# chrg127/stereomatching

Hardware: AMD Instinct MI355X
Metric: Mpixel-disparities/s (higher is better)
Workload: dtype u32 bit-packed edges, i32 counts

## Files before the change

stereomatching_amd/csrc/sm_bs_network.h:

```cpp
#pragma once

#ifdef SM_BS_NETWORK_HOST
#include <cstdint>
typedef uint32_t u32;
#define SM_NET_FN inline
#define SM_NET_UNROLL
#define SM_PIN() do { } while (0)
#define SM_SYNC() do { } while (0)
template <int IMM>
inline u32 bop(u32 a, u32 b, u32 c)
{
    u32 r = 0;
    for (int k = 0; k < 8; k++)
        if ((IMM >> k) & 1) r |= ((k & 4) ? a : ~a) & ((k & 2) ? b : ~b) & ((k & 1) ? c : ~c);
    return r;
}
#else
#define SM_NET_FN __device__ __forceinline__
#define SM_NET_UNROLL _Pragma("unroll")
#endif

#include "sm_bs_ops.h"

struct NetCell { short a, b, c, s, cy; short imm; short w; };

template <int N, int SB>
struct NetPlan {
    static constexpr int NIN = 2 * N + SB;
    static constexpr int MAXC = 2 * N + 2 * SB;
    NetCell cell[MAXC] = {};
    int ncell = 0;
    int nwires = NIN;
    int nops = 0;
    short out[SB] = {};
};

template <int N, int SB>
constexpr NetPlan<N, SB> net_make_plan()
{
    NetPlan<N, SB> p;
    short q[4 * N + 4 * SB] = {}, nx[2 * N + 2 * SB] = {};
    bool qneg[4 * N + 4 * SB] = {}, nxneg[2 * N + 2 * SB] = {};
    int head = 0, tail = 0, nn = 0;
    for (int w = 0; w < SB; w++) {
        const bool top = w == SB - 1;
        head = 0; tail = 0;
        q[tail] = (short)(2 * N + w); qneg[tail++] = false;
        if (w == 0)
            for (int i = 0; i < N; i++) {
                q[tail] = (short)i; qneg[tail++] = false;
                q[tail] = (short)(N + i); qneg[tail++] = true;
            }
        for (int i = 0; i < nn; i++) { q[tail] = nx[i]; qneg[tail++] = nxneg[i]; }
        nn = 0;
        while (tail - head >= 2) {
            const int k = tail - head >= 3 ? 3 : 2;
            short in[3] = {-1, -1, -1};
            int np = 0, ng = 0;
            for (int j = 0; j < k; j++) if (!qneg[head + j]) in[np++] = q[head + j];
            for (int j = 0; j < k; j++) if (qneg[head + j]) in[np + ng++] = q[head + j];
            head += k;
            NetCell c = {in[0], in[1], in[2], (short)p.nwires++, -1, 0, (short)w};
            bool sneg = false, cneg = false;
            if (k == 3) {
                sneg = ng & 1; cneg = ng >= 2;
                c.imm = ng == 1 ? BOP_MAJ_NC : ng == 2 ? BOP_BORROW : BOP_MAJ;
            } else {
                sneg = ng == 2; cneg = ng >= 1;
                c.imm = ng == 1 ? BOP_ANDN : 0;
            }
            p.nops++;
            if (!top) {
                c.cy = (short)p.nwires++;
                nx[nn] = c.cy; nxneg[nn++] = cneg;
                p.nops++;
            }
            q[--head] = c.s; qneg[head] = sneg;
            p.cell[p.ncell++] = c;
        }
        p.out[w] = q[head];
        if (qneg[head] && !top) { nx[nn] = q[head]; nxneg[nn++] = true; }
    }
    bool made[NetPlan<N, SB>::NIN + 2 * NetPlan<N, SB>::MAXC] = {};
    for (int i = 0; i < NetPlan<N, SB>::NIN; i++) made[i] = true;
    NetCell order[NetPlan<N, SB>::MAXC] = {};
    bool done[NetPlan<N, SB>::MAXC] = {};
    for (int n = 0; n < p.ncell; n++) {
        int pick = -1;
        for (int i = 0; i < p.ncell; i++) {
            const NetCell &c = p.cell[i];
            if (done[i] || !made[c.a] || !made[c.b] || (c.c >= 0 && !made[c.c])) continue;
            if (pick < 0 || c.w > p.cell[pick].w) pick = i;
        }
        done[pick] = true;
        order[n] = p.cell[pick];
        made[order[n].s] = true;
        if (order[n].cy >= 0) made[order[n].cy] = true;
    }
    for (int n = 0; n < p.ncell; n++) p.cell[n] = order[n];
    return p;
}

template <int N, int SB>
struct NetPlanOf { static constexpr NetPlan<N, SB> value = net_make_plan<N, SB>(); };

template <int N, int SB>
constexpr int net_min_distance(int it)
{
    const NetPlan<N, SB> p = NetPlanOf<N, SB>::value;
    int pos[NetPlan<N, SB>::NIN + 2 * NetPlan<N, SB>::MAXC] = {};
    for (int i = 0; i < NetPlan<N, SB>::NIN; i++) pos[i] = -(1 << 20);
    int at = 0, best = 1 << 20;
    for (int n = 0; n < p.ncell; n++) {
        const NetCell &c = p.cell[n];
        const short in[3] = {c.a, c.b, c.c};
        for (int j = 0; j < 3; j++)
            if (in[j] >= 0 && at - pos[in[j]] < best) best = at - pos[in[j]];
        pos[c.s] = at; at += it;
        if (c.cy >= 0) { pos[c.cy] = at; at += it; }
    }
    return best;
}

template <int N>
constexpr int net_ops() { return net_make_plan<N, bits_for(N * N)>().nops; }
constexpr int net_ops_count_tree(int n)
{
    int ops = 0, m = n;
    for (int w = 0; w < bits_for(n); w++) {
        int carries = 0;
        while (m >= 3) { ops += 2; m -= 2; carries++; }
        if (m == 2) { ops += 2; m = 1; carries++; }
        m = carries;
    }
    return ops;
}
constexpr int net_ops_addsub(int n)
{
    const int hb = bits_for(n), sb = bits_for(n * n);
    int ops = 2 + 2 * (hb - 1) + 2;
    for (int k = 1; k < sb; k++) ops += k + 1 < sb ? 2 : 1;
    return ops;
}
constexpr int net_ops_separate(int n) { return 2 * net_ops_count_tree(n) + net_ops_addsub(n); }

template <int N, int SB, int IT, int DS, int NW, int ID, typename XF>
SM_NET_FN u32 net_wire(const u32 (&S)[DS][SB], int dd0, XF &xin, const u32 (&wr)[IT][NW], int it)
{
    if constexpr (ID < 2 * N) return xin(it, ID);
    else if constexpr (ID < 2 * N + SB) return S[dd0 + it][ID - 2 * N];
    else return wr[it][ID - 2 * N - SB];
}

template <int N, int SB, int IT, int DS, int C, int NW, typename XF>
SM_NET_FN void net_cells(u32 (&S)[DS][SB], int dd0, XF &xin, u32 (&wr)[IT][NW])
{
    constexpr NetPlan<N, SB> P = NetPlanOf<N, SB>::value;
    if constexpr (C < P.ncell) {
        constexpr NetCell cl = P.cell[C];
        constexpr int NIN = 2 * N + SB;
        constexpr bool full = cl.c >= 0;
        u32 a[IT], b[IT], c[IT];
SM_NET_UNROLL
        for (int it = 0; it < IT; it++) {
            a[it] = net_wire<N, SB, IT, DS, NW, cl.a>(S, dd0, xin, wr, it);
            b[it] = net_wire<N, SB, IT, DS, NW, cl.b>(S, dd0, xin, wr, it);
            if constexpr (full) c[it] = net_wire<N, SB, IT, DS, NW, cl.c>(S, dd0, xin, wr, it);
            else c[it] = 0u;
        }
SM_NET_UNROLL
        for (int it = 0; it < IT; it++) {
            if constexpr (full) wr[it][cl.s - NIN] = bop<BOP_XOR3>(a[it], b[it], c[it]);
            else wr[it][cl.s - NIN] = a[it] ^ b[it];
            SM_PIN();
        }
        if constexpr (cl.cy >= 0) {
SM_NET_UNROLL
            for (int it = 0; it < IT; it++) {
                if constexpr (full || cl.imm != 0) wr[it][cl.cy - NIN] = bop<cl.imm>(a[it], b[it], c[it]);
                else wr[it][cl.cy - NIN] = a[it] & b[it];
                SM_PIN();
            }
        }
        SM_SYNC();
        net_cells<N, SB, IT, DS, C + 1, NW>(S, dd0, xin, wr);
    }
}

template <int N, int SB>
constexpr bool net_planes_from_cells()
{
    constexpr NetPlan<N, SB> P = NetPlanOf<N, SB>::value;
    for (int k = 0; k < SB; k++)
        if (P.out[k] < 2 * N + SB) return false;
    return true;
}

template <int N, int SB, int IT, int DS, typename XF>
SM_NET_FN void network_lockstep(u32 (&S)[DS][SB], int dd0, XF xin)
{
    constexpr NetPlan<N, SB> P = NetPlanOf<N, SB>::value;
    constexpr int NIN = 2 * N + SB, NW = P.nwires - NIN;
    static_assert(net_planes_from_cells<N, SB>(), "every plane of S' comes out of a cell");
    static_assert(net_min_distance<N, SB>(IT) >= IT, "a cell reads a result made fewer than IT operations before");
    u32 wr[IT][NW];
    net_cells<N, SB, IT, DS, 0, NW>(S, dd0, xin, wr);
SM_NET_UNROLL
    for (int k = 0; k < SB; k++)
SM_NET_UNROLL
        for (int it = 0; it < IT; it++) S[dd0 + it][k] = wr[it][P.out[k] - NIN];
}
```

stereomatching_amd/csrc/sm_match_bs_kernel.h:

```cpp

#pragma once
#include "sm_internal.h"

#ifndef SM_BS_TU
#error "define SM_BS_TU (a token naming the translation unit) before including this header"
#endif
#define SM_BS_CAT2(a, b) a##b
#define SM_BS_CAT(a, b) SM_BS_CAT2(a, b)

#define SM_BS_WAVES 2

#ifdef SM_STAMPS
static __device__ unsigned long long *g_sm_stamps;
int SM_BS_CAT(sm_bs_set_stamps_, SM_BS_TU)(void *buf)
{
    return hipMemcpyToSymbol(HIP_SYMBOL(g_sm_stamps), &buf, sizeof buf) == hipSuccess ? 0 : SM_ERR_HIP;
}
#define SM_STAMP(slot)                                                                          \
    do {                                                                                        \
        if ((threadIdx.x & 63) == 0 && g_sm_stamps) {                   \
            const size_t wg_ = (((size_t)blockIdx.z * gridDim.y + blockIdx.y) * gridDim.x + blockIdx.x) \
                               * (blockDim.x >> 6) + (threadIdx.x >> 6);                        \
            g_sm_stamps[wg_ * 10 + 2 * (slot)] = __builtin_amdgcn_s_memrealtime();              \
            g_sm_stamps[wg_ * 10 + 2 * (slot) + 1] = __builtin_amdgcn_s_memtime();              \
            if ((slot) == 0)                                                                    \
                g_sm_stamps[wg_ * 10 + 8] = ((unsigned long long)__builtin_amdgcn_s_getreg(63508) << 32) | \
                                            (unsigned)__builtin_amdgcn_s_getreg(63492);         \
        }                                                                                       \
    } while (0)
#else
#define SM_STAMP(slot) do { } while (0)
#endif

template <int IMM>
__device__ __forceinline__ u32 bop(u32 a, u32 b, u32 c)
{
    return __builtin_amdgcn_bitop3_b32(a, b, c, IMM);
}
#include "sm_bs_ops.h"

__device__ __forceinline__ u32 alignbit(u32 hi, u32 lo, u32 sh)
{
    return __builtin_amdgcn_alignbit(hi, lo, sh);
}

typedef unsigned long long u64;
struct RawRow { u64 l01; u32 l2; u64 r01, r23; };
struct RawCentre { u32 l; u64 r01; u32 r2; };
typedef __attribute__((address_space(3))) const volatile u32 lds_vu32;
typedef u64 __attribute__((aligned(4))) u64a4;
typedef __attribute__((address_space(3))) const volatile u64a4 lds_vu64;
__device__ __forceinline__ void lds_issue(RawRow &o, u32 aL, u32 aR)
{
    o.l01 = *(lds_vu64 *)(uintptr_t)aL;
    o.l2 = *(lds_vu32 *)(uintptr_t)(aL + 8);
    o.r01 = *(lds_vu64 *)(uintptr_t)aR;
    o.r23 = *(lds_vu64 *)(uintptr_t)(aR + 8);
}
__device__ __forceinline__ void lds_issue(RawCentre &o, u32 aL, u32 aR)
{
    o.l = *(lds_vu32 *)(uintptr_t)aL;
    o.r01 = *(lds_vu64 *)(uintptr_t)aR;
    o.r2 = *(lds_vu32 *)(uintptr_t)(aR + 8);
}

typedef int v4i __attribute__((ext_vector_type(4)));
__device__ __forceinline__ void store_map4(i32 *p, v4i v)
{
    asm volatile("global_store_dwordx4 %0, %1, off sc1\n\ts_nop 1" : : "v"(p), "v"(v) : "memory");
}

template <int SB, int HB>
__device__ __forceinline__ void add_planes(u32 (&s)[SB], const u32 (&h)[HB])
{
    u32 c = s[0] & h[0];
    s[0] ^= h[0];
#pragma unroll
    for (int k = 1; k < SB; k++) {
        if (k < HB) {
            const u32 cn = bop<BOP_MAJ>(s[k], h[k], c);
            s[k] = bop<BOP_XOR3>(s[k], h[k], c);
            c = cn;
        } else {
            const u32 cn = k + 1 < SB ? s[k] & c : 0u;
            s[k] ^= c;
            c = cn;
        }
    }
}

#define SM_PIN() __builtin_amdgcn_sched_barrier(0)
#define SM_SYNC() do { asm volatile("s_nop 0"); SM_PIN(); } while (0)

#include "sm_bs_network.h"

template <int N, int HB, int IT, typename XF>
__device__ __forceinline__ void count_lockstep(XF xin, u32 (&h)[IT][HB])
{
    u32 q[IT][2 * N + 2];
    int head = 0, tail = N;
#pragma unroll
    for (int w = 0; w < HB; w++) {
        u32 nx[IT][N + 1];
        int nn = 0;
#pragma unroll
        for (int adder = 0; adder < N; adder++) {
            if (tail - head >= 3) {
                u32 a[IT], b[IT], c[IT];
#pragma unroll
                for (int it = 0; it < IT; it++) {
                    const bool in0 = w == 0 && head < N, in1 = w == 0 && head + 1 < N, in2 = w == 0 && head + 2 < N;
                    a[it] = in0 ? xin(it, in0 ? head : 0) : q[it][head];
                    b[it] = in1 ? xin(it, in1 ? head + 1 : 0) : q[it][head + 1];
                    c[it] = in2 ? xin(it, in2 ? head + 2 : 0) : q[it][head + 2];
                }
#pragma unroll
                for (int it = 0; it < IT; it++) { q[it][tail] = bop<BOP_XOR3>(a[it], b[it], c[it]); SM_PIN(); }
#pragma unroll
                for (int it = 0; it < IT; it++) { nx[it][nn] = bop<BOP_MAJ>(a[it], b[it], c[it]); SM_PIN(); }
                SM_SYNC();
                head += 3; tail++; nn++;
            }
        }
        if (tail - head == 2) {
            u32 a[IT], b[IT];
#pragma unroll
            for (int it = 0; it < IT; it++) {
                const bool in0 = w == 0 && head < N, in1 = w == 0 && head + 1 < N;
                a[it] = in0 ? xin(it, in0 ? head : 0) : q[it][head];
                b[it] = in1 ? xin(it, in1 ? head + 1 : 0) : q[it][head + 1];
            }
#pragma unroll
            for (int it = 0; it < IT; it++) { q[it][tail] = a[it] ^ b[it]; SM_PIN(); }
#pragma unroll
            for (int it = 0; it < IT; it++) { nx[it][nn] = a[it] & b[it]; SM_PIN(); }
            head += 2; tail++; nn++;
        }
#pragma unroll
        for (int it = 0; it < IT; it++) {
            const bool in0 = w == 0 && head < N;
            h[it][w] = tail - head == 1 ? (in0 ? xin(it, in0 ? head : 0) : q[it][head]) : 0u;
        }
        head = 0; tail = 0;
#pragma unroll
        for (int i = 0; i < N + 1; i++)
            if (i < nn) {
#pragma unroll
                for (int it = 0; it < IT; it++) q[it][tail] = nx[it][i];
                tail++;
            }
    }
}

template <int SB, int HB, int GS, int DS>
__device__ __forceinline__ void add_lockstep(u32 (&S)[DS][SB], int dd0, const u32 (&h)[GS][HB])
{
    u32 c[GS];
#pragma unroll
    for (int g = 0; g < GS; g++) { c[g] = S[dd0 + g][0] & h[g][0]; SM_PIN(); }
#pragma unroll
    for (int g = 0; g < GS; g++) { S[dd0 + g][0] ^= h[g][0]; SM_PIN(); }
#pragma unroll
    for (int k = 1; k < SB; k++) {
        u32 cn[GS];
#pragma unroll
        for (int g = 0; g < GS; g++) {
            if (k + 1 < SB) { cn[g] = k < HB ? bop<BOP_MAJ>(S[dd0 + g][k], h[g][k], c[g]) : (S[dd0 + g][k] & c[g]); SM_PIN(); }
            else cn[g] = 0;
        }
#pragma unroll
        for (int g = 0; g < GS; g++) {
            if (k < HB) S[dd0 + g][k] = bop<BOP_XOR3>(S[dd0 + g][k], h[g][k], c[g]);
            else S[dd0 + g][k] ^= c[g];
            SM_PIN();
        }
#pragma unroll
        for (int g = 0; g < GS; g++) c[g] = cn[g];
        SM_SYNC();
    }
}

template <int V> struct IntTag { static constexpr int value = V; };

template <int CTRL>
__device__ __forceinline__ u32 dpp(u32 v)
{
    return (u32)__builtin_amdgcn_update_dpp(0, (int)v, CTRL, 0xf, 0xf, true);
}

template <int K>
__device__ __forceinline__ u32 from_partner(u32 v)
{
    if (K == 0) return dpp<0xB1>(v);
    if (K == 1) return dpp<0x4E>(v);
    if (K == 2) return dpp<0x141>(v);
    if (K == 3) return dpp<0x140>(v);
    return (u32)__shfl_xor((int)v, 1 << K);
}


template <int N, int DS, bool FULLD, bool GHOST, bool CAP2 = false, bool DUO = false>
__global__ __launch_bounds__(DUO ? 128 : 64, SM_BS_WAVES) void k_match_bs(const u32 *__restrict__ ext,
                                                 i32 *__restrict__ web, i32 *__restrict__ best,
                                                 const MatchGeom g)
{
    constexpr int HALF = N / 2;
    constexpr int HB = bits_for(N);
    constexpr int SB = bits_for(N * N);
    constexpr int AB = DS == 16 ? 4 : DS == 8 ? 3 : 2;
    constexpr int ABMAX = AB + 6;
    static_assert(SB <= 16, "window counts are moved through two byte lanes");
    static_assert((1 << SB) - 1 > N * N, "the all-ones marker must not be a real count");
    static_assert(N + DS - 1 + 31 < 96, "right window must fit three words");

    extern __shared__ __attribute__((aligned(16))) u32 lds[];
    if (CAP2) asm volatile("" ::: "v175");
    if (web == nullptr) return;
    const int tid = DUO ? (int)(threadIdx.x & 63u) : (int)threadIdx.x;
    const int wv = DUO ? __builtin_amdgcn_readfirstlane((int)(threadIdx.x >> 6)) : 0;
    const int pair = blockIdx.z;
    SM_STAMP(0);
    const unsigned slot_parity = __builtin_amdgcn_s_getreg(63492) & 1;
    unsigned long long clk = __builtin_amdgcn_s_memtime();
    constexpr unsigned PATTERN = DS == 16 ? 0xF0F0F0F0u : 0xAAAAAAAAu;
    const unsigned long long clk0 = clk;
#define SM_SLICE_PRIO()                                                               \
    do {                                                                              \
        const unsigned unit_ = (unsigned)((clk - clk0) >> 14) & 31u;                  \
        if (((PATTERN >> unit_) ^ slot_parity) & 1) __builtin_amdgcn_s_setprio(3);    \
        else __builtin_amdgcn_s_setprio(0);                                           \
    } while (0)
#define SM_SLICE_READ() do { clk = __builtin_amdgcn_s_memtime(); } while (0)
    int tile_x, tile_y;
    sm_xcd_tile(g.tiles_x, g.tiles_y, tile_x, tile_y);
    const int tx0 = tile_x * g.tw;
    const int ty0 = tile_y * (DUO ? 2 * g.tile_h : g.tile_h);
    const int plw = g.plw, prw = g.prw, nsr = g.nsr;
    const u32 *extL = ext + (size_t)pair * 2 * g.ext_image_words;
    const u32 *extR = extL + g.ext_image_words;
    u32 *pL = lds;
    u32 *pR = pL + nsr * plw;

    {
        const int wx0 = tx0 >> 5;
        const int per_row = plw + prw;
        for (int it = threadIdx.x; it < nsr * per_row; it += DUO ? 128 : 64) {
            const int row = it / per_row, k = it - row * per_row;
            const bool is_r = k >= plw;
            const int kk = is_r ? k - plw : k;
            const u32 v = (is_r ? extR : extL)[(size_t)(ty0 + row) * g.ext_words + wx0 + kk];
            if (is_r) pR[row * prw + kk] = v; else pL[row * plw + kk] = v;
        }
    }
    __syncthreads();
    SM_STAMP(1);

    const int s = tid & (g.nl - 1);
    const int wi = tid >> g.log2nl;
    const int d0 = s * DS;
    const int x0 = tx0 + 32 * wi;
    const int bL = SM_PADT + 32 * wi - HALF, bR = bL + d0;
    const int wL = bL >> 5, shL = bL & 31, wR = bR >> 5, shR = bR & 31;
    const int bRc = SM_PADT + 32 * wi + d0;
    const int wRc = bRc >> 5, shRc = bRc & 31;
    const int wLc = 1 + wi;

    u32 cvv[N];
    if (GHOST) {
        const int lo = min(64, max(0, HALF - x0)), hi = min(64, max(0, g.w + HALF - x0));
        const unsigned long long below_hi = hi >= 64 ? ~0ull : (1ull << hi) - 1ull;
        const unsigned long long below_lo = lo >= 64 ? ~0ull : (1ull << lo) - 1ull;
        const unsigned long long cm = hi > lo ? below_hi & ~below_lo : 0ull;
        const u32 c0 = (u32)cm, c1 = (u32)(cm >> 32);
#pragma unroll
        for (int i = 0; i < N; i++) cvv[i] = i ? alignbit(c1, c0, i) : c0;
    }
    u32 dvalid = (1u << DS) - 1u;
    if (!FULLD) {
        const int dlim = g.D - d0;
        dvalid = dlim >= DS ? (1u << DS) - 1u : (dlim <= 0 ? 0u : ((1u << dlim) - 1u));
    }

    u32 S[DS][SB];
#pragma unroll
    for (int dd = 0; dd < DS; dd++)
#pragma unroll
        for (int k = 0; k < SB; k++) S[dd][k] = 0;

    struct RowViews { u32 lv[N]; u32 rw[3]; };
    auto load_views = [&](int srow, RowViews &v) {
        const u32 *rl = pL + srow * plw + wL;
        const u32 *rr = pR + srow * prw + wR;
        const u32 l0 = alignbit(rl[1], rl[0], shL), l1 = alignbit(rl[2], rl[1], shL);
#pragma unroll
        for (int k = 0; k < 3; k++) v.rw[k] = alignbit(rr[k + 1], rr[k], shR);
#pragma unroll
        for (int i = 0; i < N; i++) v.lv[i] = i ? alignbit(l1, l0, i) : l0;
    };
    auto views_of = [&](const RawRow &q, RowViews &v) {
        const u32 a0 = (u32)q.l01, a1 = (u32)(q.l01 >> 32), a2 = q.l2;
        const u32 r0 = (u32)q.r01, r1 = (u32)(q.r01 >> 32), r2 = (u32)q.r23, r3 = (u32)(q.r23 >> 32);
        const u32 l0 = alignbit(a1, a0, shL), l1 = alignbit(a2, a1, shL);
        v.rw[0] = alignbit(r1, r0, shR); v.rw[1] = alignbit(r2, r1, shR); v.rw[2] = alignbit(r3, r2, shR);
#pragma unroll
        for (int i = 0; i < N; i++) v.lv[i] = i ? alignbit(l1, l0, i) : l0;
    };
    auto rview = [&](const RowViews &v, int j) -> u32 {
        return (j & 31) ? alignbit(v.rw[(j >> 5) + 1], v.rw[j >> 5], j & 31) : v.rw[j >> 5];
    };

    constexpr int GW = DS >= 4 ? 4 : DS;
    constexpr int GS = DS >= 4 ? 4 : DS;
    static_assert(DS % GW == 0 && DS % GS == 0, "shift groups");
    auto slide_in = [&](int srow) {
        RowViews v;
        load_views(srow, v);
        u32 rv[N + GW - 1];
#pragma unroll
        for (int m = 0; m < N - 1; m++) rv[m + GW] = rview(v, m);
#pragma unroll
        for (int dd0 = 0; dd0 < DS; dd0 += GW) {
#pragma unroll
            for (int m = 0; m < N - 1; m++) rv[m] = rv[m + GW];
#pragma unroll
            for (int m = 0; m < GW; m++) { rv[N - 1 + m] = rview(v, dd0 + N - 1 + m); SM_PIN(); }
            SM_SYNC();
            u32 h[GW][HB];
            count_lockstep<N, HB, GW>([&](int it, int i) -> u32 {
                const u32 x = GHOST ? bop<BOP_XOR_AND>(v.lv[i], rv[it + i], cvv[i]) : (v.lv[i] ^ rv[it + i]);
                SM_PIN();
                return x;
            }, h);
            add_lockstep<SB, HB, GW, DS>(S, dd0, h);
        }
    };
    auto slide_views = [&](const RowViews &vn, const RowViews &vo) {
        u32 rn[N + GS - 1], ro[N + GS - 1];
#pragma unroll
        for (int m = 0; m < N - 1; m++) { rn[m + GS] = rview(vn, m); ro[m + GS] = rview(vo, m); }
#pragma unroll
        for (int dd0 = 0; dd0 < DS; dd0 += GS) {
#pragma unroll
            for (int m = 0; m < N - 1; m++) { rn[m] = rn[m + GS]; ro[m] = ro[m + GS]; }
#pragma unroll
            for (int m = 0; m < GS; m++) {
                rn[N - 1 + m] = rview(vn, dd0 + N - 1 + m); SM_PIN();
                ro[N - 1 + m] = rview(vo, dd0 + N - 1 + m); SM_PIN();
            }
            SM_SYNC();
            network_lockstep<N, SB, GS, DS>(S, dd0, [&](int it, int i) -> u32 {
                const int col = i < N ? i : i - N;
                const u32 l = i < N ? vn.lv[col] : vo.lv[col];
                const u32 r = i < N ? rn[it + col] : ro[it + col];
                const u32 x = GHOST ? bop<BOP_XOR_AND>(l, r, cvv[col]) : (l ^ r);
                SM_PIN();
                return x;
            });
            SM_SYNC();
        }
    };

    const int mid = DUO ? min(ty0 + g.tile_h, g.h) : 0;
    const int sgn = DUO ? (wv ? 1 : -1) : 1;
    const int y0 = DUO ? (wv ? mid : mid - 1) : ty0;
    const int c0 = DUO ? y0 - ty0 + HALF : HALF;
    const int rows_out = DUO ? (wv ? min(ty0 + 2 * g.tile_h, g.h) - mid : mid - ty0)
                             : min(g.tile_h, g.h - ty0);

    SM_SLICE_PRIO();
    if (DUO) {
#pragma unroll 1
        for (int e = 0; e <= HALF; e++) {
        if (e == HALF) {
        constexpr int DH = DS / 2, XP = DH * SB / 2;
        static_assert(DS % 2 == 0 && (DH * SB) % 2 == 0, "exchange halves");
        typedef u32 v2u __attribute__((ext_vector_type(2)));
        v2u *xq = reinterpret_cast<v2u *>(lds + g.xm_off - XP * 128) + tid;
        auto exchange = [&](auto own_tag) {
            constexpr int OWN = decltype(own_tag)::value, OTH = 1 - OWN;
            v2u *slot_own = xq + OWN * XP * 64, *slot_oth = xq + OTH * XP * 64;
#pragma unroll
            for (int j = 0; j < XP; j++) {
                const int p = 2 * j, q = 2 * j + 1;
                const v2u v = {S[OTH * DH + p / SB][p % SB], S[OTH * DH + q / SB][q % SB]};
                slot_oth[j * 64] = v;
            }
            __syncthreads();
#pragma unroll
            for (int dd = 0; dd < DH; dd += 2) {
                u32 o[2][SB];
#pragma unroll
                for (int j = 0; j < SB; j++) {
                    const int p = 2 * j, q = 2 * j + 1;
                    const v2u v = slot_own[(dd * SB / 2 + j) * 64];
                    o[p / SB][p % SB] = v.x;
                    o[q / SB][q % SB] = v.y;
                }
                add_planes<SB, SB>(S[OWN * DH + dd], o[0]);
                add_planes<SB, SB>(S[OWN * DH + dd + 1], o[1]);
#pragma unroll
                for (int j = 0; j < SB; j++) {
                    const int p = 2 * j, q = 2 * j + 1;
                    const v2u v = {S[OWN * DH + dd + p / SB][p % SB], S[OWN * DH + dd + q / SB][q % SB]};
                    slot_own[(dd * SB / 2 + j) * 64] = v;
                }
            }
            __syncthreads();
#pragma unroll
            for (int j = 0; j < XP; j++) {
                const int p = 2 * j, q = 2 * j + 1;
                const v2u v = slot_oth[j * 64];
                S[OTH * DH + p / SB][p % SB] = v.x;
                S[OTH * DH + q / SB][q % SB] = v.y;
            }
        };
        if (wv) exchange(IntTag<1>{}); else exchange(IntTag<0>{});
        }
        slide_in(c0 + sgn * e);
        }
        if (rows_out <= 0) return;
    } else {
#pragma unroll 1
        for (int e = 0; e < N; e++) slide_in(e);
    }
    SM_SLICE_READ();
    SM_STAMP(2);

    u32 *xm_base = lds + g.xm_off - ((DUO && wv) ? g.xm_words : 0);
    u32 *xm_wbase = xm_base + (s & 3) * ((SB + AB + 3) / 4) * 256;
    const u32 xm_wunit = (u32)(wi * (g.nl >> 2) + (s >> 2) + 2 * (s & 3));
    const u32 ldsL = (u32)(uintptr_t)pL, ldsR = (u32)(uintptr_t)pR;
    const u32 sL = (u32)(sgn * 4 * plw), sR = (u32)(sgn * 4 * prw);
    u32 aNewL = ldsL + 4u * wL + sL * (HALF + 1) + 4u * plw * c0, aNewR = ldsR + 4u * wR + sR * (HALF + 1) + 4u * prw * c0;
    u32 aCenL = ldsL + 4u * wLc + 4u * plw * c0, aCenR = ldsR + 4u * wRc + 4u * prw * c0;
    RawRow qn, qo;
    RawCentre qc;
    lds_issue(qc, aCenL, aCenR);
    if (!DUO || rows_out > 1) {
        lds_issue(qn, aNewL, aNewR);
        lds_issue(qo, aNewL - sL * N, aNewR - sR * N);
    }
#pragma unroll 1
    for (int t = 0;;) {
        SM_SLICE_PRIO();
        const int y = y0 + sgn * t;
        const u32 lc = qc.l;
        const u32 c0_ = (u32)qc.r01, c1_ = (u32)(qc.r01 >> 32), c2_ = qc.r2;
        const u32 rc0 = alignbit(c1_, c0_, shRc), rc1 = alignbit(c2_, c1_, shRc);

        u32 B[SB], arg[ABMAX];
#pragma unroll
        for (int k = 0; k < ABMAX; k++) arg[k] = 0;
        {
            constexpr int Q = 4, QS = DS / Q;
            constexpr int AQ = AB - 2;
            u32 Bq[Q][SB], aq[Q][AQ > 0 ? AQ : 1];
#pragma unroll
            for (int i = 0; i < QS; i++) {
                u32 upd[Q];
                u32 rcd[Q];
#pragma unroll
                for (int qd = 0; qd < Q; qd++) {
                    const int dd = qd * QS + i;
                    rcd[qd] = dd ? alignbit(rc1, rc0, dd) : rc0; SM_PIN();
                }
                SM_SYNC();
                if (i == 0) {
#pragma unroll
                    for (int qd = 0; qd < Q; qd++) {
                        upd[qd] = bop<BOP_XNOR>(lc, rcd[qd], 0u); SM_PIN();
                        if (!FULLD) { upd[qd] &= (u32)__builtin_amdgcn_sbfe((int)dvalid, qd * QS + i, 1); SM_PIN(); }
                    }
#pragma unroll
                    for (int k = 0; k < SB; k++)
#pragma unroll
                        for (int qd = 0; qd < Q; qd++) { Bq[qd][k] = bop<BOP_ORN>(upd[qd], S[qd * QS + i][k], 0u); SM_PIN(); }
#pragma unroll
                    for (int a = 0; a < AQ; a++)
#pragma unroll
                        for (int qd = 0; qd < Q; qd++) aq[qd][a] = 0;
                } else {
                    u32 bw[Q];
#pragma unroll
                    for (int k = 0; k < SB; k++)
#pragma unroll
                        for (int qd = 0; qd < Q; qd++) {
                            bw[qd] = bop<BOP_BORROW>(Bq[qd][k], S[qd * QS + i][k], k ? bw[qd] : 0u); SM_PIN();
                            if (qd == Q - 1 && (k & 1)) SM_SYNC();
                        }
#pragma unroll
                    for (int qd = 0; qd < Q; qd++) {
                        upd[qd] = bop<BOP_UPD>(lc, rcd[qd], bw[qd]); SM_PIN();
                        if (!FULLD) { upd[qd] &= (u32)__builtin_amdgcn_sbfe((int)dvalid, qd * QS + i, 1); SM_PIN(); }
                    }
#pragma unroll
                    for (int k = 0; k < SB; k++)
#pragma unroll
                        for (int qd = 0; qd < Q; qd++) {
                            Bq[qd][k] = bop<BOP_SEL>(upd[qd], S[qd * QS + i][k], Bq[qd][k]); SM_PIN();
                            if (qd == Q - 1 && (k & 1)) SM_SYNC();
                        }
#pragma unroll
                    for (int a = 0; a < AQ; a++)
#pragma unroll
                        for (int qd = 0; qd < Q; qd++) {
                            if ((i >> a) & 1) aq[qd][a] |= upd[qd]; else aq[qd][a] = bop<BOP_ANDN>(upd[qd], aq[qd][a], 0u);
                            SM_PIN();
                        }
                }
            }
            u32 bwm[2] = {0, 0};
#pragma unroll
            for (int k = 0; k < SB; k++)
#pragma unroll
                for (int m = 0; m < 2; m++) {
                    bwm[m] = bop<BOP_BORROW>(Bq[2 * m][k], Bq[2 * m + 1][k], k ? bwm[m] : 0u); SM_PIN();
                }
            u32 Bh[2][SB], ah[2][AQ + 1];
            u32 bwf = 0;
#pragma unroll
            for (int k = 0; k < SB; k++) {
#pragma unroll
                for (int m = 0; m < 2; m++) { Bh[m][k] = bop<BOP_SEL>(bwm[m], Bq[2 * m][k], Bq[2 * m + 1][k]); SM_PIN(); }
                if (k < AQ) {
#pragma unroll
                    for (int m = 0; m < 2; m++) { ah[m][k] = bop<BOP_SEL>(bwm[m], aq[2 * m][k], aq[2 * m + 1][k]); SM_PIN(); }
                }
                if (k > 0) { bwf = bop<BOP_BORROW>(Bh[0][k - 1], Bh[1][k - 1], k > 1 ? bwf : 0u); SM_PIN(); }
            }
#pragma unroll
            for (int k = SB; k < AQ; k++)
#pragma unroll
                for (int m = 0; m < 2; m++) { ah[m][k] = bop<BOP_SEL>(bwm[m], aq[2 * m][k], aq[2 * m + 1][k]); SM_PIN(); }
            ah[0][AQ] = ~bwm[0]; SM_PIN();
            ah[1][AQ] = ~bwm[1]; SM_PIN();
            bwf = bop<BOP_BORROW>(Bh[0][SB - 1], Bh[1][SB - 1], SB > 1 ? bwf : 0u); SM_PIN();
#pragma unroll
            for (int k = 0; k < SB; k++) { B[k] = bop<BOP_SEL>(bwf, Bh[0][k], Bh[1][k]); SM_PIN(); }
#pragma unroll
            for (int k = 0; k <= AQ; k++) { arg[k] = bop<BOP_SEL>(bwf, ah[0][k], ah[1][k]); SM_PIN(); }
            arg[AQ + 1] = ~bwf; SM_PIN();
        }

        auto emit_pixels = [&](u32 (&B)[SB], u32 (&arg)[ABMAX], int xw, int yy, int pfirst, int per, int pstep) {
            const int cw = per < 4 ? per : 4;
            const u32 cmask = (1u << cw) - 1u;
            u32 allone = B[0];
#pragma unroll
            for (int k = 1; k < SB; k++) allone &= B[k];
            u32 dm1 = (u32)(g.D - 1);
            asm volatile("" : "+s"(dm1));
#pragma unroll
            for (int k = 0; k < ABMAX; k++) {
                if (k >= AB && k >= AB + g.log2nl) continue;
                arg[k] = bop<BOP_SEL>(allone, (u32)-(i32)((dm1 >> k) & 1u), arg[k]);
            }
            for (int c = 0, p0 = pfirst; c < per; c += 4, p0 += pstep) {
                u32 bb = 0, bhi = 0, alo = 0, ahi = 0;
                if (best) {
#pragma unroll
                    for (int k = 0; k < SB; k++) {
                        const u32 sp = __umul24((B[k] >> p0) & cmask, 0x204081u) & 0x01010101u;
                        if (k < 8) bb += sp << k; else bhi += sp << (k - 8);
                    }
                }
#pragma unroll
                for (int k = 0; k < ABMAX; k++) {
                    if (k >= AB && k >= AB + g.log2nl) continue;
                    const u32 sp = __umul24((arg[k] >> p0) & cmask, 0x204081u) & 0x01010101u;
                    if (k < 8) alo += sp << k; else ahi += sp << (k - 8);
                }
                const u32 none = __umul24((allone >> p0) & cmask, 0x204081u) & 0x01010101u;
                i32 wv[4], bv[4];
#pragma unroll
                for (int q = 0; q < 4; q++) {
                    const bool no = (none >> (8 * q)) & 1u;
                    int taps = N * N;
                    if (GHOST) {
                        const int x = xw + p0 + q;
                        const int cols = min(g.w - 1, x + HALF) - max(0, x - HALF) + 1;
                        const int rws = min(g.h - 1, yy + HALF) - max(0, yy - HALF) + 1;
                        taps = cols * rws;
                    }
                    const i32 a = (i32)(((alo >> (8 * q)) & 255u) | (((ahi >> (8 * q)) & 255u) << 8));
                    wv[q] = a + 1;
                    bv[q] = no ? 0 : taps - (i32)(((bb >> (8 * q)) & 255u) | (((bhi >> (8 * q)) & 255u) << 8));
                }
                const int x = xw + p0;
                const size_t o = ((size_t)pair * g.h + yy) * g.w + x;
                const bool vec = cw == 4 && g.vec_ok && x + 4 <= g.w;
                if (g.web_bytes == 4) {
                    if (vec) {
                        const v4i wq = {wv[0], wv[1], wv[2], wv[3]};
                        store_map4(web + o, wq);
                    } else {
#pragma unroll
                        for (int q = 0; q < 4; q++)
                            if (q < cw && x + q < g.w) web[o + q] = wv[q];
                    }
                } else if (g.web_bytes == 1) {
                    u8 *web8 = reinterpret_cast<u8 *>(web);
                    if (vec) {
                        u32 pk = 0;
#pragma unroll
                        for (int q = 0; q < 4; q++) pk |= (u32)(wv[q] & 255) << (8 * q);
                        __builtin_nontemporal_store(pk, reinterpret_cast<u32 *>(web8 + o));
                    } else {
#pragma unroll
                        for (int q = 0; q < 4; q++)
                            if (q < cw && x + q < g.w) web8[o + q] = (u8)wv[q];
                    }
                } else {
                    unsigned short *web16 = reinterpret_cast<unsigned short *>(web);
                    if (vec) {
                        typedef u32 v2u __attribute__((ext_vector_type(2)));
                        const v2u pk = {(u32)wv[0] | ((u32)wv[1] << 16), (u32)wv[2] | ((u32)wv[3] << 16)};
                        __builtin_nontemporal_store(pk, reinterpret_cast<v2u *>(web16 + o));
                    } else {
#pragma unroll
                        for (int q = 0; q < 4; q++)
                            if (q < cw && x + q < g.w) web16[o + q] = (unsigned short)wv[q];
                    }
                }
                if (best) {
                    if (vec) {
                        const v4i bq = {bv[0], bv[1], bv[2], bv[3]};
                        store_map4(best + o, bq);
                    } else {
#pragma unroll
                        for (int q = 0; q < 4; q++)
                            if (q < cw && x + q < g.w) best[o + q] = bv[q];
                    }
                }
            }
        };

#define SM_MERGE(K, me, NA)                                                            \
        {                                                                              \
            u32 pb[SB], pa[NA];                                                        \
            _Pragma("unroll") for (int k = 0; k < SB; k++) pb[k] = from_partner<K>(B[k]);      \
            _Pragma("unroll") for (int k = 0; k < NA; k++) pa[k] = from_partner<K>(arg[k]);    \
            SM_PIN(); SM_SYNC();                                                       \
            const u32 mine_high = ((me) >> K) & 1 ? 0xffffffffu : 0u;                  \
            u32 bw = mine_high;           \
            bw = ~bw;                       \
            _Pragma("unroll") for (int k = 0; k < SB; k++) bw = bop<BOP_BORROW>(pb[k], B[k], bw); \
            const u32 take = bw;                                                       \
            _Pragma("unroll") for (int k = 0; k < SB; k++) B[k] = bop<BOP_SEL>(take, pb[k], B[k]); \
            _Pragma("unroll") for (int k = 0; k < NA; k++) arg[k] = bop<BOP_SEL>(take, pa[k], arg[k]); \
            arg[NA] = take ^ mine_high;                 \
        }
        if (g.xmerge) {
            constexpr int NPL = SB + AB, NPG = (NPL + 3) / 4;
            typedef u32 v4u __attribute__((ext_vector_type(4)));
            typedef __attribute__((address_space(3))) const volatile v4u lds_vv4;
            const u32 xm_lds = (u32)(uintptr_t)xm_base;
            const int r = t & 3;
            {
                u32 pl[4 * NPG];
#pragma unroll
                for (int k = 0; k < 4 * NPG; k++) pl[k] = k < SB ? B[k] : (k < NPL ? arg[k - SB] : 0u);
                const u32 unit = (xm_wunit + 16u * (u32)r) & 63u;
#pragma unroll
                for (int pg = 0; pg < NPG; pg++) {
                    const v4u v = {pl[4 * pg], pl[4 * pg + 1], pl[4 * pg + 2], pl[4 * pg + 3]};
                    *reinterpret_cast<v4u *>(xm_wbase + pg * 256 + unit * 4) = v;
                }
            }
            if (r == 3 || t + 1 >= rows_out) {
                __builtin_amdgcn_fence(__ATOMIC_RELEASE, "wavefront");
                __builtin_amdgcn_wave_barrier();
                const int lpi = g.nl >> 2, l2lpi = g.log2nl - 2;
                const int rr = tid >> 4, wr = (tid & 15) >> l2lpi, sub = tid & (lpi - 1);
                u32 Bm[SB], am[ABMAX];
#pragma unroll
                for (int k = 0; k < ABMAX; k++) am[k] = 0;
                v4u ev[4][NPG];
#pragma unroll
                for (int j = 0; j < 4; j++) {
                    const u32 unit = ((u32)tid + 2u * j) & 63u;
#pragma unroll
                    for (int pg = 0; pg < NPG; pg++)
                        ev[j][pg] = *(lds_vv4 *)(uintptr_t)(xm_lds + 4u * (u32)((j * NPG + pg) * 256) + 16u * unit);
                }
                SM_PIN();
#pragma unroll
                for (int j = 0; j < 4; j++) {
                    u32 e[4 * NPG];
#pragma unroll
                    for (int pg = 0; pg < NPG; pg++) {
                        const v4u v = ev[j][pg];
                        e[4 * pg] = v.x; e[4 * pg + 1] = v.y; e[4 * pg + 2] = v.z; e[4 * pg + 3] = v.w;
                    }
                    if (j == 0) {
#pragma unroll
                        for (int k = 0; k < SB; k++) Bm[k] = e[k];
#pragma unroll
                        for (int k = 0; k < AB; k++) am[k] = e[SB + k];
                    } else {
                        u32 bw = 0xffffffffu;
#pragma unroll
                        for (int k = 0; k < SB; k++) bw = bop<BOP_BORROW>(e[k], Bm[k], bw);
                        const u32 take = bw;
#pragma unroll
                        for (int k = 0; k < SB; k++) Bm[k] = bop<BOP_SEL>(take, e[k], Bm[k]);
#pragma unroll
                        for (int k = 0; k < AB; k++) am[k] = bop<BOP_SEL>(take, e[SB + k], am[k]);
                        if (j & 1) am[AB] |= take; else am[AB] = bop<BOP_ANDN>(take, am[AB], 0u);
                        if (j & 2) am[AB + 1] |= take; else am[AB + 1] = bop<BOP_ANDN>(take, am[AB + 1], 0u);
                    }
                }
                {
                    u32 (&B)[SB] = Bm;
                    u32 (&arg)[ABMAX] = am;
                    if (lpi > 1) SM_MERGE(0, sub, AB + 2)
                    if (lpi > 2) SM_MERGE(1, sub, AB + 3)
                    if (lpi > 4) SM_MERGE(2, sub, AB + 4)
                }
                const int tt = t - r + rr;
                const int yy = y0 + sgn * tt;
                if (rr <= r && yy < g.h && yy >= 0) {
                    const int per = 32 >> l2lpi;
                    emit_pixels(Bm, am, tx0 + 32 * wr, yy, 4 * sub, per, 4 * lpi);
                }
                __builtin_amdgcn_wave_barrier();
            }
        } else {
            if (g.nl > 1) SM_MERGE(0, s, AB)
            if (g.nl > 2) SM_MERGE(1, s, AB + 1)
            if (g.nl > 4) SM_MERGE(2, s, AB + 2)
            if (g.nl > 8) SM_MERGE(3, s, AB + 3)
            if (g.nl > 16) SM_MERGE(4, s, AB + 4)
            if (g.nl > 32) SM_MERGE(5, s, AB + 5)
            if (y < g.h) {
                const int per = 32 >> g.log2nl;
                emit_pixels(B, arg, x0, y, s * per, per, 4);
            }
        }
#undef SM_MERGE

        SM_SYNC();
        if (++t >= rows_out) break;
        {
            RowViews vn, vo;
            views_of(qn, vn);
            views_of(qo, vo);
            aNewL += sL; aNewR += sR; aCenL += sL; aCenR += sR;
            lds_issue(qc, aCenL, aCenR);
            if (t + 1 < rows_out) {
                lds_issue(qn, aNewL, aNewR);
                lds_issue(qo, aNewL - sL * N, aNewR - sR * N);
            }
            SM_SLICE_READ();
            SM_PIN(); SM_SYNC();
            slide_views(vn, vo);
        }
    }
    SM_STAMP(3);
}


template <int N, int DS, bool CAP2, bool DUO = false>
static const void *bs_ptr4(bool fulld, bool ghost)
{
    return fulld ? (ghost ? (const void *)k_match_bs<N, DS, true, true, CAP2, DUO> : (const void *)k_match_bs<N, DS, true, false, CAP2, DUO>)
                 : (ghost ? (const void *)k_match_bs<N, DS, false, true, CAP2, DUO> : (const void *)k_match_bs<N, DS, false, false, CAP2, DUO>);
}
template <int N, int DS, bool CAPPABLE>
static const void *bs_ptr(bool fulld, bool ghost, bool cap2)
{
    if (cap2) return CAPPABLE ? bs_ptr4<N, DS, CAPPABLE>(fulld, ghost) : nullptr;
    return bs_ptr4<N, DS, false>(fulld, ghost);
}
```

Measured before the change: 11.94 million.

## Group census inputs in threes to share XOR3 parity across disparities

```diff
diff --git a/stereomatching_amd/csrc/sm_bs_network.h b/stereomatching_amd/csrc/sm_bs_network.h
--- a/stereomatching_amd/csrc/sm_bs_network.h
+++ b/stereomatching_amd/csrc/sm_bs_network.h
@@ -22,7 +22,7 @@
 
 #include "sm_bs_ops.h"
 
-struct NetCell { short a, b, c, s, cy; short imm; short w; };
+struct NetCell { short a, b, c, s, cy; short imm; short w; bool grp = false; };
 
 template <int N, int SB>
 struct NetPlan {
@@ -35,26 +35,44 @@
     short out[SB] = {};
 };
 
-template <int N, int SB>
+template <int N, int SB, bool GR = false>
 constexpr NetPlan<N, SB> net_make_plan()
 {
     NetPlan<N, SB> p;
+    constexpr int G = GR ? N / 3 : 0;
     short q[4 * N + 4 * SB] = {}, nx[2 * N + 2 * SB] = {};
     bool qneg[4 * N + 4 * SB] = {}, nxneg[2 * N + 2 * SB] = {};
+    short qgrp[4 * N + 4 * SB] = {};
     int head = 0, tail = 0, nn = 0;
     for (int w = 0; w < SB; w++) {
         const bool top = w == SB - 1;
         head = 0; tail = 0;
         q[tail] = (short)(2 * N + w); qneg[tail++] = false;
-        if (w == 0)
-            for (int i = 0; i < N; i++) {
+        if (w == 0) {
+            for (int g = 0; g < G; g++) {
+                qgrp[tail] = (short)(1 + 3 * g); qneg[tail++] = false;
+                qgrp[tail] = (short)(1 + N + 3 * g); qneg[tail++] = true;
+            }
+            for (int i = 3 * G; i < N; i++) {
                 q[tail] = (short)i; qneg[tail++] = false;
                 q[tail] = (short)(N + i); qneg[tail++] = true;
             }
+        }
         for (int i = 0; i < nn; i++) { q[tail] = nx[i]; qneg[tail++] = nxneg[i]; }
         nn = 0;
         while (tail - head >= 2) {
             const int k = tail - head >= 3 ? 3 : 2;
+            for (int j = 0; j < k; j++)
+                if (qgrp[head + j]) {
+                    const short in0 = (short)(qgrp[head + j] - 1);
+                    NetCell gc = {in0, (short)(in0 + 1), (short)(in0 + 2), -1, -1, BOP_MAJ_NC, (short)w, true};
+                    gc.s = (short)p.nwires++;
+                    gc.cy = (short)p.nwires++;
+                    nx[nn] = gc.cy; nxneg[nn++] = qneg[head + j];
+                    p.nops++;
+                    q[head + j] = gc.s; qgrp[head + j] = 0;
+                    p.cell[p.ncell++] = gc;
+                }
             short in[3] = {-1, -1, -1};
             int np = 0, ng = 0;
             for (int j = 0; j < k; j++) if (!qneg[head + j]) in[np++] = q[head + j];
@@ -101,13 +119,13 @@
     return p;
 }
 
-template <int N, int SB>
-struct NetPlanOf { static constexpr NetPlan<N, SB> value = net_make_plan<N, SB>(); };
-
-template <int N, int SB>
+template <int N, int SB, bool GR = false>
+struct NetPlanOf { static constexpr NetPlan<N, SB> value = net_make_plan<N, SB, GR>(); };
+
+template <int N, int SB, bool GR = false>
 constexpr int net_min_distance(int it)
 {
-    const NetPlan<N, SB> p = NetPlanOf<N, SB>::value;
+    const NetPlan<N, SB> p = NetPlanOf<N, SB, GR>::value;
     int pos[NetPlan<N, SB>::NIN + 2 * NetPlan<N, SB>::MAXC] = {};
     for (int i = 0; i < NetPlan<N, SB>::NIN; i++) pos[i] = -(1 << 20);
     int at = 0, best = 1 << 20;
@@ -116,14 +134,15 @@
         const short in[3] = {c.a, c.b, c.c};
         for (int j = 0; j < 3; j++)
             if (in[j] >= 0 && at - pos[in[j]] < best) best = at - pos[in[j]];
-        pos[c.s] = at; at += it;
+        pos[c.s] = at;
+        if (!c.grp) at += it;
         if (c.cy >= 0) { pos[c.cy] = at; at += it; }
     }
     return best;
 }
 
-template <int N>
-constexpr int net_ops() { return net_make_plan<N, bits_for(N * N)>().nops; }
+template <int N, bool GR = false>
+constexpr int net_ops() { return net_make_plan<N, bits_for(N * N), GR>().nops; }
 constexpr int net_ops_count_tree(int n)
 {
     int ops = 0, m = n;
@@ -152,10 +171,10 @@
     else return wr[it][ID - 2 * N - SB];
 }
 
-template <int N, int SB, int IT, int DS, int C, int NW, typename XF>
+template <int N, int SB, int IT, int DS, bool GR, int C, int NW, typename XF>
 SM_NET_FN void net_cells(u32 (&S)[DS][SB], int dd0, XF &xin, u32 (&wr)[IT][NW])
 {
-    constexpr NetPlan<N, SB> P = NetPlanOf<N, SB>::value;
+    constexpr NetPlan<N, SB> P = NetPlanOf<N, SB, GR>::value;
     if constexpr (C < P.ncell) {
         constexpr NetCell cl = P.cell[C];
         constexpr int NIN = 2 * N + SB;
@@ -170,9 +189,12 @@
         }
 SM_NET_UNROLL
         for (int it = 0; it < IT; it++) {
-            if constexpr (full) wr[it][cl.s - NIN] = bop<BOP_XOR3>(a[it], b[it], c[it]);
-            else wr[it][cl.s - NIN] = a[it] ^ b[it];
-            SM_PIN();
+            if constexpr (cl.grp) wr[it][cl.s - NIN] = c[it];
+            else {
+                if constexpr (full) wr[it][cl.s - NIN] = bop<BOP_XOR3>(a[it], b[it], c[it]);
+                else wr[it][cl.s - NIN] = a[it] ^ b[it];
+                SM_PIN();
+            }
         }
         if constexpr (cl.cy >= 0) {
 SM_NET_UNROLL
@@ -183,28 +205,28 @@
             }
         }
         SM_SYNC();
-        net_cells<N, SB, IT, DS, C + 1, NW>(S, dd0, xin, wr);
-    }
-}
-
-template <int N, int SB>
+        net_cells<N, SB, IT, DS, GR, C + 1, NW>(S, dd0, xin, wr);
+    }
+}
+
+template <int N, int SB, bool GR = false>
 constexpr bool net_planes_from_cells()
 {
-    constexpr NetPlan<N, SB> P = NetPlanOf<N, SB>::value;
+    constexpr NetPlan<N, SB> P = NetPlanOf<N, SB, GR>::value;
     for (int k = 0; k < SB; k++)
         if (P.out[k] < 2 * N + SB) return false;
     return true;
 }
 
-template <int N, int SB, int IT, int DS, typename XF>
+template <int N, int SB, int IT, int DS, bool GR = false, typename XF>
 SM_NET_FN void network_lockstep(u32 (&S)[DS][SB], int dd0, XF xin)
 {
-    constexpr NetPlan<N, SB> P = NetPlanOf<N, SB>::value;
+    constexpr NetPlan<N, SB> P = NetPlanOf<N, SB, GR>::value;
     constexpr int NIN = 2 * N + SB, NW = P.nwires - NIN;
-    static_assert(net_planes_from_cells<N, SB>(), "every plane of S' comes out of a cell");
-    static_assert(net_min_distance<N, SB>(IT) >= IT, "a cell reads a result made fewer than IT operations before");
+    static_assert(net_planes_from_cells<N, SB, GR>(), "every plane of S' comes out of a cell");
+    static_assert(net_min_distance<N, SB, GR>(IT) >= IT, "a cell reads a result made fewer than IT operations before");
     u32 wr[IT][NW];
-    net_cells<N, SB, IT, DS, 0, NW>(S, dd0, xin, wr);
+    net_cells<N, SB, IT, DS, GR, 0, NW>(S, dd0, xin, wr);
 SM_NET_UNROLL
     for (int k = 0; k < SB; k++)
 SM_NET_UNROLL
diff --git a/stereomatching_amd/csrc/sm_match_bs_kernel.h b/stereomatching_amd/csrc/sm_match_bs_kernel.h
--- a/stereomatching_amd/csrc/sm_match_bs_kernel.h
+++ b/stereomatching_amd/csrc/sm_match_bs_kernel.h
@@ -334,10 +334,26 @@
             add_lockstep<SB, HB, GW, DS>(S, dd0, h);
         }
     };
+    constexpr int G = N / 3, RXK = 3 * (G - 1), RXW = RXK + GS;
+    constexpr bool GROUPED = !GHOST && 2 * G * DS > 2 * G + 2 * (RXK + DS) && !(DS == 8 && N >= 19);
     auto slide_views = [&](const RowViews &vn, const RowViews &vo) {
         u32 rn[N + GS - 1], ro[N + GS - 1];
+        u32 lxn[G], lxo[G], rxn[RXW], rxo[RXW];
 #pragma unroll
         for (int m = 0; m < N - 1; m++) { rn[m + GS] = rview(vn, m); ro[m + GS] = rview(vo, m); }
+        if (GROUPED) {
+            SM_PIN(); SM_SYNC();
+#pragma unroll
+            for (int gq = 0; gq < G; gq++) {
+                lxn[gq] = bop<BOP_XOR3>(vn.lv[3 * gq], vn.lv[3 * gq + 1], vn.lv[3 * gq + 2]); SM_PIN();
+                lxo[gq] = bop<BOP_XOR3>(vo.lv[3 * gq], vo.lv[3 * gq + 1], vo.lv[3 * gq + 2]); SM_PIN();
+            }
+#pragma unroll
+            for (int m = 0; m < RXK; m++) {
+                rxn[m + GS] = bop<BOP_XOR3>(rn[m + GS], rn[m + GS + 1], rn[m + GS + 2]); SM_PIN();
+                rxo[m + GS] = bop<BOP_XOR3>(ro[m + GS], ro[m + GS + 1], ro[m + GS + 2]); SM_PIN();
+            }
+        }
 #pragma unroll
         for (int dd0 = 0; dd0 < DS; dd0 += GS) {
 #pragma unroll
@@ -348,8 +364,21 @@
                 ro[N - 1 + m] = rview(vo, dd0 + N - 1 + m); SM_PIN();
             }
             SM_SYNC();
-            network_lockstep<N, SB, GS, DS>(S, dd0, [&](int it, int i) -> u32 {
+            if (GROUPED) {
+#pragma unroll
+                for (int m = 0; m < RXK; m++) { rxn[m] = rxn[m + GS]; rxo[m] = rxo[m + GS]; }
+#pragma unroll
+                for (int m = 0; m < GS; m++) { rxn[RXK + m] = bop<BOP_XOR3>(rn[RXK + m], rn[RXK + m + 1], rn[RXK + m + 2]); SM_PIN(); }
+#pragma unroll
+                for (int m = 0; m < GS; m++) { rxo[RXK + m] = bop<BOP_XOR3>(ro[RXK + m], ro[RXK + m + 1], ro[RXK + m + 2]); SM_PIN(); }
+            }
+            network_lockstep<N, SB, GS, DS, GROUPED>(S, dd0, [&](int it, int i) -> u32 {
                 const int col = i < N ? i : i - N;
+                if (GROUPED && col < 3 * G && col % 3 == 2) {
+                    const u32 p = (i < N ? lxn[col / 3] : lxo[col / 3]) ^ (i < N ? rxn[it + col - 2] : rxo[it + col - 2]);
+                    SM_PIN();
+                    return p;
+                }
                 const u32 l = i < N ? vn.lv[col] : vo.lv[col];
                 const u32 r = i < N ? rn[it + col] : ro[it + col];
                 const u32 x = GHOST ? bop<BOP_XOR_AND>(l, r, cvv[col]) : (l ^ r);
```

Measured after the change: 12.16 million, median of 6. 1.8% higher.
